# jlko/STOVE

Hardware: AMD Instinct MI355X
Metric: frames/s (fwd+bwd) for 3-obj billiards 32x32 T=100, 1/2/4/8 GPU; ELBO delta vs ref (higher is better)
Workload: dtype f32 (encoder GEMMs: fp32 products as 3 sixteen-bit MFMAs on hi/lo-split operands -- half pieces forward, bf16 pieces backward -- fp32 accumulate)

## Files before the change

### stove_amd/csrc/capi.hip

```cpp
#include "../../include/stove_hip.h"
#include <algorithm>

#include "common.h"
#include <string.h>
#include <stdlib.h>
#include <math.h>
#include <atomic>
#include <type_traits>
#include "validate.h"
static_assert(stove_validate::kStoveInvalidValue == (int)hipErrorInvalidValue, "validate.h returns hipErrorInvalidValue");
#define STOVE_VALIDATE(expr)                      \
  do {                                            \
    const int v__ = stove_validate::expr;         \
    if (v__) return v__;                          \
  } while (0)
#include "spn_obj.hip"
#include "spn_obj_generic.hip"
#include "spn_bg.hip"
#include "spn_bg_generic.hip"
#include "scene.hip"
#include "scene_fused.hip"
#include "scene_colour.hip"
#include "gnn.hip"
#include "match.hip"
// ... 1266 lines not shown
  *graph_out = (void*)g;
  return (int)e;
}

int stove_graph_instantiate(void* graph, void** exec_out) {
  if (exec_out == nullptr) return (int)hipErrorInvalidValue;
  *exec_out = nullptr;
  if (graph == nullptr) return 0;
  hipGraph_t g = (hipGraph_t)graph;
  size_t n = 0;
  hipError_t e = hipGraphGetNodes(g, nullptr, &n);
  if (e == hipSuccess && n > 0) {
    hipGraphExec_t x = nullptr;
    e = hipGraphInstantiate(&x, g, nullptr, nullptr, 0);
    if (e == hipSuccess) *exec_out = (void*)x;
  }
  const hipError_t d = hipGraphDestroy(g);
  return (int)(e != hipSuccess ? e : d);
}

int stove_graph_launch(void* exec, void* stream) { return (int)hipGraphLaunch((hipGraphExec_t)exec, (hipStream_t)stream); }

int stove_graph_destroy(void* exec) { return exec == nullptr ? 0 : (int)hipGraphExecDestroy((hipGraphExec_t)exec); }

int stove_bw_transform(const float* x, float* out, int n_frames, int channels, int pixels, void* stream) {
  if (n_frames == 0) return 0;
  if (pixels % 4 != 0 || channels < 1) return (int)hipErrorInvalidValue;
  const long long total = (long long)n_frames * (pixels / 4);
  if (total > 0x7fffffffLL) return (int)hipErrorInvalidValue;
  STOVE_LAUNCH(bw_transform_k, dim3((unsigned)((total + 255) / 256)), dim3(256), 0, (hipStream_t)stream, x, out, n_frames, channels, pixels / 4);
  STOVE_LAUNCH_CHECK();
  return 0;
}

int stove_bw_transform_u8(const unsigned char* x, float* out, int n_frames, int channels, int pixels, void* stream) {
  if (n_frames == 0) return 0;
  if (pixels % 4 != 0 || channels < 1) return (int)hipErrorInvalidValue;
  const long long total = (long long)n_frames * (pixels / 4);
  if (total > 0x7fffffffLL) return (int)hipErrorInvalidValue;
  STOVE_LAUNCH(bw_transform_u8_k, dim3((unsigned)((total + 255) / 256)), dim3(256), 0, (hipStream_t)stream, x, out, n_frames, channels, pixels / 4);
  STOVE_LAUNCH_CHECK();
  return 0;
}

size_t stove_colsum_ws_floats(int rows, int cols) {
  const int chunks = rows < 512 ? (rows < 1 ? 1 : rows) : 512;
  return (size_t)(chunks + 16) * cols;
}

static int colsum_level(const float* a, float* part, int rows, int cols, int max_chunks, hipStream_t st) {
  const int chunks = rows < max_chunks ? rows : max_chunks;
  const int per = (rows + chunks - 1) / chunks;
  const int used = (rows + per - 1) / per;
  if (cols <= 64) {
    int cpad = 1;
    while (cpad < cols) cpad <<= 1;
    STOVE_LAUNCH(colsum_narrow_part_k, dim3(used), dim3(256), 0, st, a, part, rows, cols, cpad, per);
  } else {
    STOVE_LAUNCH(colsum_part_k, dim3(used, (cols / 4 + 255) / 256), dim3(256), 0, st, a, part, rows, cols / 4, per);
  }
  return used;
}

int stove_colsum(const float* a, float* out, float* ws, int rows, int cols, void* stream) { return stove_colsum2(a, out, nullptr, 0, ws, rows, cols, stream); }

int stove_colsum2(const float* a, float* out, float* out2, int accumulate, float* ws, int rows, int cols, void* stream) {
  hipStream_t st = (hipStream_t)stream;
  if (cols <= 0 || (cols % 4 != 0 && cols > 64)) return (int)hipErrorInvalidValue;
  if (rows == 0) {
    if (!accumulate) {
      hipMemsetAsync(out, 0, sizeof(float) * cols, st);
      if (out2 != nullptr) hipMemsetAsync(out2, 0, sizeof(float) * cols, st);
    }
    return 0;
  }
  int used = colsum_level(a, ws, rows, cols, 512, st);
  STOVE_LAUNCH_CHECK();
  const float* src = ws;
  if (used > 16) {
    float* ws2 = ws + (size_t)(rows < 512 ? rows : 512) * cols;
    used = colsum_level(ws, ws2, used, cols, 16, st);
    STOVE_LAUNCH_CHECK();
    src = ws2;
  }
  STOVE_LAUNCH(reduce_chunks_k, dim3((cols + 31) / 32), dim3(256), 0, st, src, out, cols, used, accumulate, out2);
  STOVE_LAUNCH_CHECK();
  return 0;
}

static int small_tn_chunks(int rows) { return rows < 64 ? 1 : (rows / 64 < 512 ? rows / 64 : 512); }
size_t stove_small_tn_ws_floats(int rows, int M, int N) { return (size_t)small_tn_chunks(rows) * M * N; }

int stove_small_tn(const float* a, const float* b, float* out, float* ws, int rows, int M, int N, void* stream) {
  hipStream_t st = (hipStream_t)stream;
  if (M < 1 || N < 1 || M * N > 256) return (int)hipErrorInvalidValue;
  if (rows == 0) {
    hipMemsetAsync(out, 0, sizeof(float) * M * N, st);
    return 0;
  }
  const int chunks = small_tn_chunks(rows), per = (rows + chunks - 1) / chunks;
  STOVE_LAUNCH(small_tn_part_k, dim3(chunks), dim3(256), 0, st, a, b, ws, rows, M, N, per);
  STOVE_LAUNCH_CHECK();
  STOVE_LAUNCH(reduce_chunks_k, dim3((M * N + 31) / 32), dim3(256), 0, st, (const float*)ws, out, M * N, chunks, 0);
  STOVE_LAUNCH_CHECK();
  return 0;
}

size_t stove_flat_adam_ws_bytes(int nseg) { return (size_t)nseg * sizeof(int) + ADAM_SCAN_BLOCKS * sizeof(float); }

int stove_flat_adam(float* params, const float* grads, float* exp_avg, float* exp_avg_sq, float* max_exp_avg_sq, size_t numel,
                    const int* seg_of4, const unsigned char* seg_trainable, float* seg_steps, int nseg, void* ws, float* grad_norm_out,
                    const float* hyper_dev, float lr, float beta1, float beta2, float eps, float max_norm, int clip, void* stream) {
  if (numel == 0 || nseg == 0) return 0;
  if (numel % 4 != 0 || ws == nullptr || seg_of4 == nullptr || seg_trainable == nullptr || seg_steps == nullptr)
    return (int)hipErrorInvalidValue;
  AdamHyper k;
  k.lr = lr; k.b1 = beta1; k.b2 = beta2; k.eps = eps; k.max_norm = max_norm;
  const int n4 = (int)(numel / 4);
  hipStream_t st = (hipStream_t)stream;
  float* part = reinterpret_cast<float*>(ws);
  int* flags = reinterpret_cast<int*>(part + ADAM_SCAN_BLOCKS);
  STOVE_LAUNCH(grad_scan_k, dim3(ADAM_SCAN_BLOCKS), dim3(256), 0, st, grads, seg_of4, flags, part, n4);
  STOVE_LAUNCH(flat_adam_k, dim3((n4 + 255) / 256), dim3(256), 0, st, params, grads, exp_avg, exp_avg_sq, max_exp_avg_sq, seg_of4,
               seg_trainable, (const float*)seg_steps, (const int*)flags, (const float*)part, grad_norm_out, hyper_dev, k, clip & 1, n4);
  STOVE_LAUNCH(adam_tick_k, dim3((nseg + 255) / 256), dim3(256), 0, st, seg_trainable, seg_steps, flags, nseg, (clip >> 1) & 1);
  STOVE_LAUNCH_CHECK();
  return 0;
}

static ZpConst zp_const(const float* span_low) {
  ZpConst k;
  for (int d = 0; d < 8; ++d) {
    k.span[d] = span_low[d];
    k.low[d] = span_low[8 + d];
  }
  return k;
}

int stove_supair_state_fwd(const float* codes, const float* span_low, float* zc, float* pos, long long* idx, float* zfix,
                           unsigned char* hits, float* zl, float* sl, float* init6, int n, int T, int o, int skip, int fix,
                           int mode, void* stream) {
  return stove_supair_state_fwd2(codes, span_low, zc, pos, idx, zfix, hits, zl, sl, init6, 6, nullptr, 0, n, T, o, skip, fix, mode, stream);
}

int stove_supair_state_fwd2(const float* codes, const float* span_low, float* zc, float* pos, long long* idx, float* zfix,
                            unsigned char* hits, float* zl, float* sl, float* init, int init_ld, const float* lat_noise, int lat_dim,
                            int n, int T, int o, int skip, int fix, int mode, void* stream) {
  if (init_ld < 6 + (lat_noise != nullptr ? lat_dim : 0) || lat_dim < 0) return (int)hipErrorInvalidValue;
  float* init6 = init;
  hipStream_t st = (hipStream_t)stream;
  if (n == 0) return 0;
  if (T < 2 || skip < 1 || skip >= T || o < 1 || o > kMatchN) return (int)hipErrorInvalidValue;
  const int M = n * T * o;
  if (codes != nullptr) {
    STOVE_LAUNCH(zp_constrain_k, dim3((M * 8 + 255) / 256), dim3(256), 0, st, codes, zp_const(span_low), zc, pos, M);
    STOVE_LAUNCH_CHECK();
    int rc = stove_match_objects(pos, idx, nullptr, n, T, o, 2, mode, stream);
    if (rc) return rc;
  }
  STOVE_LAUNCH(supair_state_fwd_k, dim3((M + 255) / 256), dim3(256), 0, st, (const float*)zc, (const long long*)idx, zfix, hits, zl, sl,
               init6, n, T, o, skip, fix, init_ld, lat_noise, lat_dim);
  STOVE_LAUNCH_CHECK();
  return 0;
}

int stove_supair_state_bwd(const float* zc, const long long* idx, const unsigned char* hits, const float* zfix, const float* g_zfix,
                           const float* g_zl, const float* g_sl, const float* g_init6, const float* span_low, float* gfix_ws,
                           float* g_codes, int n, int T, int o, int skip, void* stream) {
  return stove_supair_state_bwd2(zc, idx, hits, zfix, g_zfix, g_zl, g_sl, g_init6, 6, span_low, gfix_ws, g_codes, n, T, o, skip, stream);
}

int stove_supair_state_bwd2(const float* zc, const long long* idx, const unsigned char* hits, const float* zfix, const float* g_zfix,
                            const float* g_zl, const float* g_sl, const float* g_init6, int init_ld, const float* span_low, float* gfix_ws,
                            float* g_codes, int n, int T, int o, int skip, void* stream) {
  hipStream_t st = (hipStream_t)stream;
  if (n == 0) return 0;
  const int M = n * T * o;
  (void)gfix_ws;
  STOVE_LAUNCH(supair_state_bwd_k, dim3((M + 255) / 256), dim3(256), 0, st, zc, idx, hits, zfix, g_zfix, g_zl, g_sl, g_init6, zp_const(span_low),
               g_codes, n, T, o, skip, init_ld);
  STOVE_LAUNCH_CHECK();
  return 0;
}

int stove_noise_normal(float* out, size_t n, unsigned long long* state, void* stream) {
  if (n == 0) return 0;
  if (((uintptr_t)out & 15) != 0 || state == nullptr) return (int)hipErrorInvalidValue;
  const size_t threads = (n + 3) / 4;
  if ((threads + 255) / 256 > 0x7fffffffULL) return (int)hipErrorInvalidValue;
  STOVE_LAUNCH(noise_normal_k, dim3((unsigned)((threads + 255) / 256)), dim3(256), 0, (hipStream_t)stream, out, n, (const unsigned long long*)state);
  STOVE_LAUNCH(noise_tick_k, dim3(1), dim3(1), 0, (hipStream_t)stream, state);
  STOVE_LAUNCH_CHECK();
  return 0;
}

int stove_zall_fwd(const float* zfix, const float* zs, float* zall, int n, int T, int o, int skip, void* stream) {
  if (n == 0) return 0;
  const int M = n * (T - 1) * o;
  STOVE_LAUNCH(zall_fwd_k, dim3((M + 255) / 256), dim3(256), 0, (hipStream_t)stream, zfix, zs, zall, n, T, o, skip);
  STOVE_LAUNCH_CHECK();
  return 0;
}

int stove_zall_bwd(const float* zfix, const float* zs, const float* g_zall, const float* dz_in, float* g_zfix, float* g_zs, int n, int T, int o,
                   int skip, void* stream) {
  if (n == 0) return 0;
  const int M = n * T * o + n * (T - skip) * o;
  STOVE_LAUNCH(zall_bwd_k, dim3((M + 255) / 256), dim3(256), 0, (hipStream_t)stream, zfix, zs, g_zall, dz_in, g_zfix, g_zs, n, T, o, skip);
  STOVE_LAUNCH_CHECK();
  return 0;
}

static TransStd trans_std(const float* s16) {
  TransStd t;
  for (int d = 0; d < 16; ++d) t.s[d] = s16[d];
  return t;
}

int stove_elbo_fwd(const float* zs, const float* mean, const float* std_, const float* zdyn, const float* lik, const float* trans_std16,
                   float* part_ws, float* out3, int n, int T, int o, int skip, void* stream) {
  hipStream_t st = (hipStream_t)stream;
  if (n == 0 || skip < 1 || skip >= T) return (int)hipErrorInvalidValue;
  STOVE_LAUNCH(elbo_part_k, dim3(n), dim3(256), 0, st, zs, mean, std_, zdyn, lik, trans_std(trans_std16), part_ws, T, o, skip);
  STOVE_LAUNCH_CHECK();
  STOVE_LAUNCH(elbo_final_k, dim3(1), dim3(256), 0, st, (const float*)part_ws, out3, n, T, skip);
  STOVE_LAUNCH_CHECK();
  return 0;
}

int stove_elbo_bwd(const float* zs, const float* mean, const float* std_, const float* zdyn, const float* trans_std16, const float* g_out,
                   float* g_zs, float* g_mean, float* g_std, float* g_zdyn, float* g_lik, int n, int T, int o, int skip, void* stream) {
  if (n == 0) return 0;
  const size_t M = (size_t)n * (T - skip) * o * 18 + (size_t)n * (T - 1);
  STOVE_LAUNCH(elbo_bwd_k, dim3((unsigned)((M + 255) / 256)), dim3(256), 0, (hipStream_t)stream, zs, mean, std_, zdyn, trans_std(trans_std16), g_out,
               g_zs, g_mean, g_std, g_zdyn, g_lik, n, T, o, skip);
  STOVE_LAUNCH_CHECK();
  return 0;
}

static int enc_head_groups(int rows) {
  const int tiles = (rows + 15) / 16;
  int g = (tiles + 3) / 4;
  return g < 1 ? 1 : (g > 102 ? 102 : g);
}

int stove_enc_head_fwd(const float* h, const float* W1, const float* b1, const float* W2, const float* b2, float* h1, float* codes, int rows,
                       int H, int HID, int OUT, int frames, int fc1_split, void* stream) {
  if (H != kEhH || HID < 1 || HID > kEhHid || OUT != kEhOut || frames < 0 || (frames > 0 && rows % frames != 0)) return (int)hipErrorInvalidValue;
  if (rows == 0) return 0;
  static_assert(2 * kEhHid * kEhLdB == sizeof(float) * kEhHid * kEhLd, "the two bf16 images of W1 take the fp32 image's place");
  const size_t lds = sizeof(float) * kEhHid * kEhLd;
  const int tiles = (rows + 15) / 16;
  const int grid = (tiles + 3) / 4 < 512 ? (tiles + 3) / 4 : 512;
  int rc;
  if (fc1_split) {
    rc = (int)hipFuncSetAttribute((const void*)enc_head_fwd_k<true>, hipFuncAttributeMaxDynamicSharedMemorySize, (int)lds);
    if (rc) return rc;
    STOVE_LAUNCH((enc_head_fwd_k<true>), dim3(grid), dim3(256), lds, (hipStream_t)stream, h, W1, b1, W2, b2, h1, codes, rows, HID, frames);
  } else {
    rc = (int)hipFuncSetAttribute((const void*)enc_head_fwd_k<false>, hipFuncAttributeMaxDynamicSharedMemorySize, (int)lds);
    if (rc) return rc;
    STOVE_LAUNCH((enc_head_fwd_k<false>), dim3(grid), dim3(256), lds, (hipStream_t)stream, h, W1, b1, W2, b2, h1, codes, rows, HID, frames);
  }
  STOVE_LAUNCH_CHECK();
  return 0;
}

size_t stove_enc_head_bwd_ws_floats(int rows, int HID) { return (size_t)enc_head_groups(rows) * eh_part_floats(HID); }

int stove_enc_head_bwd(const float* dcodes, const float* h1, const float* h, const float* W1, const float* W2, float* gh, float* gW1,
                       float* gb1, float* gW2, float* gb2, int accumulate, float* ws, int rows, int H, int HID, int OUT, int frames, void* stream) {
  if (H != kEhH || HID < 1 || HID > kEhHid || OUT != kEhOut || frames < 0 || (frames > 0 && rows % frames != 0)) return (int)hipErrorInvalidValue;
  hipStream_t st = (hipStream_t)stream;
  const int P = eh_part_floats(HID);
  if (rows == 0) {
    if (!accumulate) {
      hipMemsetAsync(gW1, 0, sizeof(float) * HID * kEhH, st);
      hipMemsetAsync(gW2, 0, sizeof(float) * kEhOut * HID, st);
      hipMemsetAsync(gb1, 0, sizeof(float) * HID, st);
      hipMemsetAsync(gb2, 0, sizeof(float) * kEhOut, st);
    }
    return 0;
  }
  const int groups = enc_head_groups(rows);
  const size_t lds = sizeof(float) * kEhBwdLds;
  int rc;
  if (HID <= 50) {
    rc = (int)hipFuncSetAttribute((const void*)enc_head_bwd_k<14>, hipFuncAttributeMaxDynamicSharedMemorySize, (int)lds);
    if (rc) return rc;
    STOVE_LAUNCH(enc_head_bwd_k<14>, dim3(groups * 5), dim3(256), lds, st, dcodes, h1, h, W1, W2, gh, ws, rows, HID, groups, frames);
  } else {
    rc = (int)hipFuncSetAttribute((const void*)enc_head_bwd_k<16>, hipFuncAttributeMaxDynamicSharedMemorySize, (int)lds);
    if (rc) return rc;
    STOVE_LAUNCH(enc_head_bwd_k<16>, dim3(groups * 5), dim3(256), lds, st, dcodes, h1, h, W1, W2, gh, ws, rows, HID, groups, frames);
  }
  STOVE_LAUNCH_CHECK();
  (void)P;
  STOVE_LAUNCH(enc_head_reduce_k, dim3((eh_part_floats(HID) + 31) / 32), dim3(256), 0, st, (const float*)ws, gW1, gW2, gb1, gb2, HID, groups, accumulate);
  STOVE_LAUNCH_CHECK();
  return 0;
}

int stove_lstm_cell_fwd(const float* gx, const float* gh, const float* c_prev, float* c, float* h, int n, int H, int fast, void* stream) {
  if (n == 0) return 0;
  if (H % 4) return (int)hipErrorInvalidValue;
  const size_t total = (size_t)n * (H / 4);
// ... 116 lines not shown
```

### stove_amd/csrc/match.hip

```cpp
#include "common.h"

namespace stove {

constexpr int kMatchN = 8, kMatchF = 8;

template <int TN, int TF>
__global__ __launch_bounds__(64) void match_objects_k(const float* __restrict__ feat, long long* __restrict__ idx_out,
                                                      float* __restrict__ perm_out, int B, int T, int Nrt, int Frt, int mode) {
  const int N = TN > 0 ? TN : Nrt;
  const int F = TF > 0 ? TF : Frt;
  extern __shared__ float mlds[];
  const int b = blockIdx.x;
  const int n_feat = T * N * F;
  int* ibuf = reinterpret_cast<int*>(mlds + n_feat);
  for (int i = threadIdx.x; i < n_feat; i += 64) mlds[i] = feat[(size_t)b * n_feat + i];
  __syncthreads();
  if (threadIdx.x == 0) {
  constexpr int MN = TN > 0 ? TN : kMatchN, MF = TF > 0 ? TF : kMatchF;
  float prev[MN][MF], cur[MN][MF], err[MN][MN];
  const float* fb = mlds;
  _Pragma("unroll") for (int a = 0; a < N; ++a) {
    _Pragma("unroll") for (int f = 0; f < F; ++f) prev[a][f] = (fb[a * F + f] + 1.0f) * 0.5f;
    ibuf[a] = a;
  }
// ... 156 lines not shown
    e = fmaf(d, d, e);
  }
  return e;
}
__device__ __forceinline__ bool greedy_rounds(float (&e)[kMatchN][kMatchN], int N, int* assign) {
  bool tie = false;
  for (int round = 0; round < N; ++round) {
    float bv = __builtin_inff();
    int ba = 0, bj = 0, cnt = 0;
#pragma unroll
    for (int a = 0; a < kMatchN; ++a)
#pragma unroll
      for (int j = 0; j < kMatchN; ++j) {
        if (a < N && j < N) {
          const float v = e[a][j];
          cnt = v < bv ? 1 : (v == bv ? cnt + 1 : cnt);
          if (v < bv) {
            bv = v;
            ba = a;
            bj = j;
          }
        }
      }
    tie = tie || (cnt > 1 && bv < 3.0e38f);
    assign[ba] = bj;
#pragma unroll
    for (int a = 0; a < kMatchN; ++a)
#pragma unroll
      for (int j = 0; j < kMatchN; ++j)
        if (a == ba || j == bj) e[a][j] = 3.0e38f;
  }
  return tie;
}
__device__ __forceinline__ unsigned char* greedy_scratch(long long* idx_out, int b, int T, int N) {
  return reinterpret_cast<unsigned char*>(idx_out + (size_t)(b + 1) * T * N) - (size_t)T * N - T;
}
__global__ __launch_bounds__(256) void match_greedy_frames_k(const float* __restrict__ feat, long long* __restrict__ idx_out, int B, int T, int N, int F) {
  const int i = blockIdx.x * blockDim.x + threadIdx.x;
  if (i >= B * T) return;
  const int b = i / T, t = i % T;
  unsigned char* sc = greedy_scratch(idx_out, b, T, N);
  if (t == 0) {
    for (int a = 0; a < N; ++a) sc[a] = (unsigned char)a;
    sc[(size_t)T * N] = 0;
    return;
  }
  const float* prev = feat + ((size_t)b * T + t - 1) * N * F;
  const float* cur = prev + (size_t)N * F;
  float e[kMatchN][kMatchN];
#pragma unroll
  for (int a = 0; a < kMatchN; ++a)
#pragma unroll
    for (int j = 0; j < kMatchN; ++j) e[a][j] = (a < N && j < N) ? match_err(prev + a * F, cur + j * F, F) : 3.0e38f;
  int assign[kMatchN];
#pragma unroll
  for (int a = 0; a < kMatchN; ++a) assign[a] = 0;
  const bool tie = greedy_rounds(e, N, assign);
#pragma unroll
  for (int a = 0; a < kMatchN; ++a)
    if (a < N) sc[(size_t)t * N + a] = (unsigned char)assign[a];
  sc[(size_t)T * N + t] = tie ? 1 : 0;
}
__global__ __launch_bounds__(64) void match_greedy_compose_k(const float* __restrict__ feat, long long* __restrict__ idx_out, int B, int T, int N, int F) {
  extern __shared__ unsigned char glds[];
  const int b = blockIdx.x, lane = threadIdx.x;
  const unsigned char* sc = greedy_scratch(idx_out, b, T, N);
  const int nsc = T * N + T;
  for (int i = lane; i < nsc; i += 64) glds[i] = sc[i];
  int* ibuf = reinterpret_cast<int*>(glds + ((nsc + 3) & ~3));
  __shared__ int slot[kMatchN];
  __syncthreads();
  int r = lane < N ? lane : 0;
  if (lane < N) ibuf[lane] = r;
  for (int t = 1; t < T; ++t) {
    if (glds[T * N + t] == 0) {
      r = glds[t * N + r];
    } else {
      if (lane < N) slot[lane] = r;
      __syncthreads();
      if (lane == 0) {
        const float* prev = feat + ((size_t)b * T + t - 1) * N * F;
        const float* cur = prev + (size_t)N * F;
        float e[kMatchN][kMatchN];
#pragma unroll
        for (int a = 0; a < kMatchN; ++a)
#pragma unroll
          for (int j = 0; j < kMatchN; ++j) e[a][j] = (a < N && j < N) ? match_err(prev + slot[a < N ? a : 0] * F, cur + j * F, F) : 3.0e38f;
        int assign[kMatchN];
#pragma unroll
        for (int a = 0; a < kMatchN; ++a) assign[a] = 0;
        greedy_rounds(e, N, assign);
#pragma unroll
        for (int a = 0; a < kMatchN; ++a)
          if (a < N) slot[a] = assign[a];
      }
      __syncthreads();
      if (lane < N) r = slot[lane];
      __syncthreads();
    }
    if (lane < N) ibuf[t * N + lane] = r;
  }
  __syncthreads();
  for (int i = lane; i < T * N; i += 64) idx_out[(size_t)b * T * N + i] = ibuf[i];
}

struct Perm3 {
  int p0, p1, p2;
};
__device__ __forceinline__ Perm3 perm3_of(int k) {
  Perm3 r;
  r.p0 = k >> 1;
  const int lo = r.p0 == 0 ? 1 : 0, hi = r.p0 == 2 ? 1 : 2;
  r.p1 = (k & 1) ? hi : lo;
  r.p2 = (k & 1) ? lo : hi;
  return r;
}
__device__ __forceinline__ int perm3_id(const Perm3& p) { return 2 * p.p0 + (p.p1 > p.p2 ? 1 : 0); }
__device__ __forceinline__ float sel3(int i, float a, float b, float c) { return i == 0 ? a : (i == 1 ? b : c); }
__device__ __forceinline__ Perm3 match3_step(const float (&D)[3][3], const Perm3& p) {
  float e[3][3];
#pragma unroll
  for (int j = 0; j < 3; ++j) {
    e[0][j] = sel3(p.p0, D[0][j], D[1][j], D[2][j]);
    e[1][j] = sel3(p.p1, D[0][j], D[1][j], D[2][j]);
    e[2][j] = sel3(p.p2, D[0][j], D[1][j], D[2][j]);
  }
  int idx[3];
#pragma unroll
  for (int a = 0; a < 3; ++a) {
    int best = 0;
    if (e[a][1] < e[a][best]) best = 1;
    if (e[a][2] < sel3(best, e[a][0], e[a][1], e[a][2])) best = 2;
    idx[a] = best;
  }
  if (idx[0] == idx[1] || idx[0] == idx[2] || idx[1] == idx[2]) {
#pragma unroll
    for (int a = 0; a < 3; ++a) {
      int best = 0;
      if (e[a][1] < e[a][0]) best = 1;
      if (e[a][2] < sel3(best, e[a][0], e[a][1], e[a][2])) best = 2;
      idx[a] = best;
#pragma unroll
      for (int r = 0; r < 3; ++r) {
        e[r][0] = best == 0 ? 1e12f : e[r][0];
        e[r][1] = best == 1 ? 1e12f : e[r][1];
        e[r][2] = best == 2 ? 1e12f : e[r][2];
      }
    }
  }
  return Perm3{idx[0], idx[1], idx[2]};
}

template <int F>
__global__ __launch_bounds__(64) void match3_table_k(const float* __restrict__ feat, long long* __restrict__ idx_out, int B, int T) {
  extern __shared__ float mlds[];
  const int b = blockIdx.x, lane = threadIdx.x;
  const int n_feat = T * 3 * F;
  int* ibuf = reinterpret_cast<int*>(mlds + n_feat);
  for (int i = lane; i < n_feat; i += 64) mlds[i] = feat[(size_t)b * n_feat + i];
  __syncthreads();
  const int chunk = (T - 1 + 63) / 64;
  const int t0 = 1 + lane * chunk, t1 = t0 + chunk < T ? t0 + chunk : T;
  auto table = [&](int t, float (&D)[3][3]) {
    float pv[3][F], cv[3][F];
#pragma unroll
    for (int i = 0; i < 3; ++i)
#pragma unroll
      for (int f = 0; f < F; ++f) {
        pv[i][f] = (mlds[((t - 1) * 3 + i) * F + f] + 1.0f) * 0.5f;
        cv[i][f] = (mlds[(t * 3 + i) * F + f] + 1.0f) * 0.5f;
      }
#pragma unroll
    for (int i = 0; i < 3; ++i)
#pragma unroll
      for (int j = 0; j < 3; ++j) {
        float sacc = 0.0f;
#pragma unroll
        for (int f = 0; f < F; ++f) {
          const float d = pv[i][f] - cv[j][f];
          sacc += d * d;
        }
        D[i][j] = sacc;
      }
  };
  int cur[6] = {0, 1, 2, 3, 4, 5};
  for (int t = t0; t < t1; ++t) {
    float D[3][3];
    table(t, D);
#pragma unroll
    for (int k = 0; k < 6; ++k) cur[k] = perm3_id(match3_step(D, perm3_of(cur[k])));
  }
  unsigned m = 0;
#pragma unroll
  for (int k = 0; k < 6; ++k) m |= (unsigned)cur[k] << (3 * k);
#pragma unroll
  for (int d = 1; d < 64; d <<= 1) {
    const unsigned o = (unsigned)__builtin_amdgcn_ds_bpermute(((lane - d) & 63) * 4, (int)m);
    if (lane >= d) {
      unsigned n = 0;
#pragma unroll
      for (int k = 0; k < 6; ++k) n |= ((m >> (3 * ((o >> (3 * k)) & 7u))) & 7u) << (3 * k);
      m = n;
    }
  }
  const unsigned before = (unsigned)__builtin_amdgcn_ds_bpermute(((lane - 1) & 63) * 4, (int)m);
  Perm3 p = perm3_of(lane == 0 ? 0 : (int)(before & 7u));
  if (lane == 0) {
    ibuf[0] = 0;
    ibuf[1] = 1;
    ibuf[2] = 2;
  }
  for (int t = t0; t < t1; ++t) {
    float D[3][3];
    table(t, D);
    p = match3_step(D, p);
    ibuf[t * 3 + 0] = p.p0;
    ibuf[t * 3 + 1] = p.p1;
    ibuf[t * 3 + 2] = p.p2;
  }
  __syncthreads();
  for (int i = lane; i < T * 3; i += 64) idx_out[(size_t)b * T * 3 + i] = ibuf[i];
}

}
```

### stove_amd/csrc/state.hip

```cpp
#include "common.h"

namespace stove {

struct ZpConst {
  float span[8], low[8];
};

__global__ void zp_constrain_k(const float* __restrict__ codes, ZpConst kc, float* __restrict__ zc, float* __restrict__ pos, int M) {
  const int i = blockIdx.x * blockDim.x + threadIdx.x;
  if (i >= M * 8) return;
  const int d = i & 7;
  const float v = fmaf(kc.span[d], sigmoidf_(codes[i]), kc.low[d]);
  zc[i] = v;
  if (d == 2 || d == 3) pos[(i >> 3) * 2 + d - 2] = v;
}

__device__ __forceinline__ void load8(const float* __restrict__ p, float* v) {
  const float4 a = *reinterpret_cast<const float4*>(p), b = *reinterpret_cast<const float4*>(p + 4);
  v[0] = a.x; v[1] = a.y; v[2] = a.z; v[3] = a.w; v[4] = b.x; v[5] = b.y; v[6] = b.z; v[7] = b.w;
}

__device__ __forceinline__ int fixed_state(const float* __restrict__ zc, const long long* __restrict__ idx, int b, int t, int k, int T,
                                           int o, int fix, float* out) {
  const size_t row = (size_t)b * T + t;
  float cur[8];
  load8(zc + (row * o + idx[row * o + k]) * 8, cur);
  int hit = 0;
  if (fix && t >= 1 && t <= T - 2) {
    float pv[8], nx[8];
    load8(zc + ((row - 1) * o + idx[(row - 1) * o + k]) * 8, pv);
    load8(zc + ((row + 1) * o + idx[(row + 1) * o + k]) * 8, nx);
#pragma unroll
    for (int a = 0; a < 2; ++a)
      if (fabsf(cur[a] - pv[a]) > 0.095f && fabsf(nx[a] - cur[a]) > 0.095f) hit |= 1 << a;
#pragma unroll
    for (int d = 0; d < 8; ++d)
      if (hit & (1 << (d & 1))) cur[d] = 0.5f * (pv[d] + nx[d]);
  }
#pragma unroll
  for (int d = 0; d < 8; ++d) out[d] = cur[d];
  return hit;
}

__global__ void supair_state_fwd_k(const float* __restrict__ zc, const long long* __restrict__ idx, float* __restrict__ zfix,
                                   unsigned char* __restrict__ hits, float* __restrict__ zl, float* __restrict__ sl,
                                   float* __restrict__ init6, int n, int T, int o, int skip, int fix, int init_ld,
                                   const float* __restrict__ lat_noise, int lat_dim) {
  const int i = blockIdx.x * blockDim.x + threadIdx.x;
  if (i >= n * T * o) return;
  const int k = i % o, t = (i / o) % T, b = i / (o * T);
  float cur[8], pv[8];
  const int hit = fixed_state(zc, idx, b, t, k, T, o, fix, cur);
  hits[i] = (unsigned char)hit;
#pragma unroll
  for (int d = 0; d < 8; ++d) zfix[(size_t)i * 8 + d] = cur[d];
  if (t < skip - 1 || t < 1) return;
  fixed_state(zc, idx, b, t - 1, k, T, o, fix, pv);
  float z6[6], s6[6];
#pragma unroll
  for (int d = 0; d < 4; ++d) {
    z6[d] = cur[d];
    s6[d] = cur[4 + d];
  }
#pragma unroll
  for (int a = 0; a < 2; ++a) {
    z6[4 + a] = cur[2 + a] - pv[2 + a];
    s6[4 + a] = sqrtf(cur[6 + a] * cur[6 + a] + pv[6 + a] * pv[6 + a]);
  }
  if (t == skip - 1) {
#pragma unroll
    for (int d = 0; d < 6; ++d) init6[((size_t)b * o + k) * init_ld + d] = z6[d];
    if (lat_noise != nullptr)
      for (int d = 0; d < lat_dim; ++d) init6[((size_t)b * o + k) * init_ld + 6 + d] = 0.01f * lat_noise[((size_t)b * o + k) * lat_dim + d];
  } else {
    const size_t r = (((size_t)b * (T - skip) + (t - skip)) * o + k) * 6;
#pragma unroll
    for (int d = 0; d < 6; ++d) {
      zl[r + d] = z6[d];
      sl[r + d] = s6[d];
    }
  }
}

__device__ __forceinline__ void g6_at(const float* __restrict__ g_zl, const float* __restrict__ g_sl, const float* __restrict__ g_init6,
                                      int b, int t, int k, int T, int o, int skip, float* gz, float* gs, int init_ld) {
#pragma unroll
  for (int d = 0; d < 6; ++d) gz[d] = gs[d] = 0.0f;
  if (t < 1 || t > T - 1) return;
  if (t == skip - 1) {
    if (g_init6 != nullptr)
#pragma unroll
      for (int d = 0; d < 6; ++d) gz[d] = g_init6[((size_t)b * o + k) * init_ld + d];
  } else if (t >= skip) {
    const size_t r = (((size_t)b * (T - skip) + (t - skip)) * o + k) * 6;
#pragma unroll
    for (int d = 0; d < 6; ++d) {
      if (g_zl != nullptr) gz[d] = g_zl[r + d];
      if (g_sl != nullptr) gs[d] = g_sl[r + d];
    }
  }
}

__device__ __forceinline__ void supair_gfix(const float* __restrict__ zfix, const float* __restrict__ g_zfix, const float* __restrict__ g_zl,
                                            const float* __restrict__ g_sl, const float* __restrict__ g_init6, size_t i, int T, int o, int skip,
                                            int init_ld, float (&g)[8]) {
  const int k = (int)(i % o), t = (int)((i / o) % T), b = (int)(i / ((size_t)o * T));
#pragma unroll
  for (int d = 0; d < 8; ++d) g[d] = g_zfix != nullptr ? g_zfix[i * 8 + d] : 0.0f;
  float gz[6], gs[6], gzn[6], gsn[6];
  g6_at(g_zl, g_sl, g_init6, b, t, k, T, o, skip, gz, gs, init_ld);
  g6_at(g_zl, g_sl, g_init6, b, t + 1, k, T, o, skip, gzn, gsn, init_ld);
#pragma unroll
  for (int d = 0; d < 4; ++d) {
    g[d] += gz[d];
    g[4 + d] += gs[d];
  }
  float cur[8];
  load8(zfix + i * 8, cur);
#pragma unroll
  for (int a = 0; a < 2; ++a) {
    g[2 + a] += gz[4 + a] - gzn[4 + a];
    if (gs[4 + a] != 0.0f) {
      const float p = zfix[(i - o) * 8 + 6 + a];
      g[6 + a] += gs[4 + a] * cur[6 + a] / sqrtf(cur[6 + a] * cur[6 + a] + p * p);
    }
    if (gsn[4 + a] != 0.0f) {
      const float q = zfix[(i + o) * 8 + 6 + a];
      g[6 + a] += gsn[4 + a] * cur[6 + a] / sqrtf(q * q + cur[6 + a] * cur[6 + a]);
    }
  }
}

__global__ void supair_state_bwd_k(const float* __restrict__ zc, const long long* __restrict__ idx, const unsigned char* __restrict__ hits,
                                   const float* __restrict__ zfix, const float* __restrict__ g_zfix, const float* __restrict__ g_zl,
                                   const float* __restrict__ g_sl, const float* __restrict__ g_init6, ZpConst kc, float* __restrict__ g_codes,
                                   int n, int T, int o, int skip, int init_ld) {
  const int i = blockIdx.x * blockDim.x + threadIdx.x;
  if (i >= n * T * o) return;
  const int j = i % o, t = (i / o) % T, b = i / (o * T);
  const size_t row = (size_t)b * T + t;
  float acc[8] = {0, 0, 0, 0, 0, 0, 0, 0};
  for (int k = 0; k < o; ++k) {
    if ((int)idx[row * o + k] != j) continue;
    const size_t e = row * o + k;
    const int h0 = hits[e];
    const int hp = (t >= 1) ? hits[e - o] : 0, hn = (t <= T - 2) ? hits[e + o] : 0;
    float g0[8], gp[8], gn[8];
    supair_gfix(zfix, g_zfix, g_zl, g_sl, g_init6, e, T, o, skip, init_ld, g0);
    if (hp) supair_gfix(zfix, g_zfix, g_zl, g_sl, g_init6, e - o, T, o, skip, init_ld, gp);
    if (hn) supair_gfix(zfix, g_zfix, g_zl, g_sl, g_init6, e + o, T, o, skip, init_ld, gn);
#pragma unroll
    for (int d = 0; d < 8; ++d) {
      const int bit = 1 << (d & 1);
      float v = (h0 & bit) ? 0.0f : g0[d];
      if (hp & bit) v += 0.5f * gp[d];
      if (hn & bit) v += 0.5f * gn[d];
      acc[d] += v;
    }
  }
#pragma unroll
  for (int d = 0; d < 8; ++d) {
    const float s = (zc[(size_t)i * 8 + d] - kc.low[d]) / kc.span[d];
    g_codes[(size_t)i * 8 + d] = acc[d] * kc.span[d] * s * (1.0f - s);
  }
}

__global__ void zall_fwd_k(const float* __restrict__ zfix, const float* __restrict__ zs, float* __restrict__ zall, int n, int T, int o, int skip) {
  const int i = blockIdx.x * blockDim.x + threadIdx.x;
  if (i >= n * (T - 1) * o) return;
  const int k = i % o, j = (i / o) % (T - 1), b = i / (o * (T - 1));
  const float* src = (j < skip - 1) ? zfix + (((size_t)b * T + 1 + j) * o + k) * 8 : zs + (((size_t)b * (T - skip) + (j - (skip - 1))) * o + k) * 18;
  const float sx = src[0];
  zall[(size_t)i * 4] = sx;
  zall[(size_t)i * 4 + 1] = sx * src[1];
  zall[(size_t)i * 4 + 2] = src[2];
  zall[(size_t)i * 4 + 3] = src[3];
}
__global__ void zall_bwd_k(const float* __restrict__ zfix, const float* __restrict__ zs, const float* __restrict__ g_zall,
                           const float* __restrict__ dz_in, float* __restrict__ g_zfix, float* __restrict__ g_zs, int n, int T, int o, int skip) {
  const int i = blockIdx.x * blockDim.x + threadIdx.x;
  const int nfix = n * T * o, nzs = n * (T - skip) * o;
  if (i < nfix) {
    const int k = i % o, t = (i / o) % T, b = i / (o * T);
    float g[8] = {0, 0, 0, 0, 0, 0, 0, 0};
    if (t >= 1 && t < skip) {
      const size_t a = (((size_t)b * (T - 1) + (t - 1)) * o + k) * 4;
      const float* src = zfix + (size_t)i * 8;
      g[0] = g_zall[a] + g_zall[a + 1] * src[1];
      g[1] = g_zall[a + 1] * src[0];
      g[2] = g_zall[a + 2];
      g[3] = g_zall[a + 3];
    }
#pragma unroll
    for (int d = 0; d < 8; ++d) g_zfix[(size_t)i * 8 + d] = g[d];
  } else if (i < nfix + nzs) {
    const int q = i - nfix;
    const int k = q % o, ts = (q / o) % (T - skip), b = q / (o * (T - skip));
    const size_t a = (((size_t)b * (T - 1) + (skip - 1 + ts)) * o + k) * 4;
    const float* src = zs + (size_t)q * 18;
    float* g = g_zs + (size_t)q * 18;
    float v[4];
    v[0] = g_zall[a] + g_zall[a + 1] * src[1];
    v[1] = g_zall[a + 1] * src[0];
    v[2] = g_zall[a + 2];
    v[3] = g_zall[a + 3];
    if (dz_in == nullptr) {
#pragma unroll
      for (int d = 0; d < 18; ++d) g[d] = d < 4 ? v[d] : 0.0f;
    } else {
      const float* gi = dz_in + (size_t)q * 18;
#pragma unroll
      for (int d = 0; d < 18; ++d) g[d] = d < 4 ? v[d] + gi[d] : gi[d];
    }
  }
}

__device__ __forceinline__ void philox_round(uint32_t& c0, uint32_t& c1, uint32_t& c2, uint32_t& c3, uint32_t k0, uint32_t k1) {
  const uint64_t p0 = (uint64_t)0xD2511F53u * c0, p1 = (uint64_t)0xCD9E8D57u * c2;
  const uint32_t n0 = (uint32_t)(p1 >> 32) ^ c1 ^ k0, n2 = (uint32_t)(p0 >> 32) ^ c3 ^ k1;
  c1 = (uint32_t)p1;
  c3 = (uint32_t)p0;
  c0 = n0;
  c2 = n2;
}
__device__ __forceinline__ float u01(uint32_t r) { return ((float)(r >> 8) + 0.5f) * (1.0f / 16777216.0f); }
__global__ __launch_bounds__(256) void noise_normal_k(float* __restrict__ out, size_t n, const unsigned long long* __restrict__ state) {
  const size_t i = (size_t)blockIdx.x * blockDim.x + threadIdx.x;
  if (4 * i >= n) return;
  const unsigned long long seed = state[0], call = state[1];
  uint32_t c0 = (uint32_t)call, c1 = (uint32_t)(call >> 32), c2 = (uint32_t)i, c3 = (uint32_t)(i >> 32);
  uint32_t k0 = (uint32_t)seed, k1 = (uint32_t)(seed >> 32);
#pragma unroll
  for (int r = 0; r < 10; ++r) {
// ... 108 lines not shown
```

Measured before the change: 9.099 million.

## Fuse zp constrain, 3-object matching and state fwd into one per-sequence kernel

For the 3-object, mode-0 case, a single kernel per batch element now computes the sigmoid constraint on the codes, keeps zc and pos in LDS, runs the 3-object table match walk on one wavefront, and builds the fixed states from LDS. Before, this took three separate launches with global round-trips for zc, pos and idx. The match walk is factored into a shared device function, and the state element code is templated on the index type so it can read the int LDS buffer. The cost is one block per sequence with only 64 of 256 threads active during matching, which may lower parallelism for small n.

```diff
diff --git a/stove_amd/csrc/capi.hip b/stove_amd/csrc/capi.hip
--- a/stove_amd/csrc/capi.hip
+++ b/stove_amd/csrc/capi.hip
@@ -1442,6 +1442,12 @@
   if (n == 0) return 0;
   if (T < 2 || skip < 1 || skip >= T || o < 1 || o > kMatchN) return (int)hipErrorInvalidValue;
   const int M = n * T * o;
+  if (codes != nullptr && mode == 0 && o == 3 && state3_lds_bytes(T) <= 64 * 1024) {
+    STOVE_LAUNCH(supair_state3_fwd_k, dim3(n), dim3(kState3Threads), state3_lds_bytes(T), st, codes, zp_const(span_low), zc, pos, idx, zfix, hits,
+                 zl, sl, init6, T, skip, fix, init_ld, lat_noise, lat_dim);
+    STOVE_LAUNCH_CHECK();
+    return 0;
+  }
   if (codes != nullptr) {
     STOVE_LAUNCH(zp_constrain_k, dim3((M * 8 + 255) / 256), dim3(256), 0, st, codes, zp_const(span_low), zc, pos, M);
     STOVE_LAUNCH_CHECK();
diff --git a/stove_amd/csrc/match.hip b/stove_amd/csrc/match.hip
--- a/stove_amd/csrc/match.hip
+++ b/stove_amd/csrc/match.hip
@@ -332,13 +332,7 @@
 }
 
 template <int F>
-__global__ __launch_bounds__(64) void match3_table_k(const float* __restrict__ feat, long long* __restrict__ idx_out, int B, int T) {
-  extern __shared__ float mlds[];
-  const int b = blockIdx.x, lane = threadIdx.x;
-  const int n_feat = T * 3 * F;
-  int* ibuf = reinterpret_cast<int*>(mlds + n_feat);
-  for (int i = lane; i < n_feat; i += 64) mlds[i] = feat[(size_t)b * n_feat + i];
-  __syncthreads();
+__device__ __forceinline__ void match3_table_walk(const float* mlds, int* ibuf, int T, int lane) {
   const int chunk = (T - 1 + 63) / 64;
   const int t0 = 1 + lane * chunk, t1 = t0 + chunk < T ? t0 + chunk : T;
   auto table = [&](int t, float (&D)[3][3]) {
@@ -398,6 +392,17 @@
     ibuf[t * 3 + 1] = p.p1;
     ibuf[t * 3 + 2] = p.p2;
   }
+}
+
+template <int F>
+__global__ __launch_bounds__(64) void match3_table_k(const float* __restrict__ feat, long long* __restrict__ idx_out, int B, int T) {
+  extern __shared__ float mlds[];
+  const int b = blockIdx.x, lane = threadIdx.x;
+  const int n_feat = T * 3 * F;
+  int* ibuf = reinterpret_cast<int*>(mlds + n_feat);
+  for (int i = lane; i < n_feat; i += 64) mlds[i] = feat[(size_t)b * n_feat + i];
+  __syncthreads();
+  match3_table_walk<F>(mlds, ibuf, T, lane);
   __syncthreads();
   for (int i = lane; i < T * 3; i += 64) idx_out[(size_t)b * T * 3 + i] = ibuf[i];
 }
diff --git a/stove_amd/csrc/state.hip b/stove_amd/csrc/state.hip
--- a/stove_amd/csrc/state.hip
+++ b/stove_amd/csrc/state.hip
@@ -20,7 +20,8 @@
   v[0] = a.x; v[1] = a.y; v[2] = a.z; v[3] = a.w; v[4] = b.x; v[5] = b.y; v[6] = b.z; v[7] = b.w;
 }
 
-__device__ __forceinline__ int fixed_state(const float* __restrict__ zc, const long long* __restrict__ idx, int b, int t, int k, int T,
+template <typename IdxT>
+__device__ __forceinline__ int fixed_state(const float* __restrict__ zc, const IdxT* __restrict__ idx, int b, int t, int k, int T,
                                            int o, int fix, float* out) {
   const size_t row = (size_t)b * T + t;
   float cur[8];
@@ -42,20 +43,19 @@
   return hit;
 }
 
-__global__ void supair_state_fwd_k(const float* __restrict__ zc, const long long* __restrict__ idx, float* __restrict__ zfix,
-                                   unsigned char* __restrict__ hits, float* __restrict__ zl, float* __restrict__ sl,
-                                   float* __restrict__ init6, int n, int T, int o, int skip, int fix, int init_ld,
-                                   const float* __restrict__ lat_noise, int lat_dim) {
-  const int i = blockIdx.x * blockDim.x + threadIdx.x;
-  if (i >= n * T * o) return;
-  const int k = i % o, t = (i / o) % T, b = i / (o * T);
+template <typename IdxT>
+__device__ __forceinline__ void supair_state_elem(const float* __restrict__ zc, const IdxT* __restrict__ idx, int bz, int b, int t, int k,
+                                                  float* __restrict__ zfix, unsigned char* __restrict__ hits, float* __restrict__ zl,
+                                                  float* __restrict__ sl, float* __restrict__ init6, int T, int o, int skip, int fix,
+                                                  int init_ld, const float* __restrict__ lat_noise, int lat_dim) {
+  const size_t i = ((size_t)b * T + t) * o + k;
   float cur[8], pv[8];
-  const int hit = fixed_state(zc, idx, b, t, k, T, o, fix, cur);
+  const int hit = fixed_state(zc, idx, bz, t, k, T, o, fix, cur);
   hits[i] = (unsigned char)hit;
 #pragma unroll
-  for (int d = 0; d < 8; ++d) zfix[(size_t)i * 8 + d] = cur[d];
+  for (int d = 0; d < 8; ++d) zfix[i * 8 + d] = cur[d];
   if (t < skip - 1 || t < 1) return;
-  fixed_state(zc, idx, b, t - 1, k, T, o, fix, pv);
+  fixed_state(zc, idx, bz, t - 1, k, T, o, fix, pv);
   float z6[6], s6[6];
 #pragma unroll
   for (int d = 0; d < 4; ++d) {
@@ -79,6 +79,50 @@
       zl[r + d] = z6[d];
       sl[r + d] = s6[d];
     }
+  }
+}
+
+__global__ void supair_state_fwd_k(const float* __restrict__ zc, const long long* __restrict__ idx, float* __restrict__ zfix,
+                                   unsigned char* __restrict__ hits, float* __restrict__ zl, float* __restrict__ sl,
+                                   float* __restrict__ init6, int n, int T, int o, int skip, int fix, int init_ld,
+                                   const float* __restrict__ lat_noise, int lat_dim) {
+  const int i = blockIdx.x * blockDim.x + threadIdx.x;
+  if (i >= n * T * o) return;
+  const int k = i % o, t = (i / o) % T, b = i / (o * T);
+  supair_state_elem(zc, idx, b, b, t, k, zfix, hits, zl, sl, init6, T, o, skip, fix, init_ld, lat_noise, lat_dim);
+}
+
+constexpr int kState3Threads = 256;
+__host__ __device__ inline size_t state3_lds_bytes(int T) { return (size_t)T * 3 * (8 + 2 + 1) * sizeof(float); }
+__global__ __launch_bounds__(kState3Threads) void supair_state3_fwd_k(const float* __restrict__ codes, ZpConst kc, float* __restrict__ zc,
+                                                                      float* __restrict__ pos, long long* __restrict__ idx_out,
+                                                                      float* __restrict__ zfix, unsigned char* __restrict__ hits,
+                                                                      float* __restrict__ zl, float* __restrict__ sl,
+                                                                      float* __restrict__ init6, int T, int skip, int fix, int init_ld,
+                                                                      const float* __restrict__ lat_noise, int lat_dim) {
+  extern __shared__ __attribute__((aligned(16))) float s3_lds[];
+  float* zc_s = s3_lds;
+  float* pos_s = zc_s + T * 3 * 8;
+  int* ibuf = reinterpret_cast<int*>(pos_s + T * 3 * 2);
+  const int b = blockIdx.x, tid = threadIdx.x;
+  const int M = T * 3;
+  const size_t row0 = (size_t)b * M;
+  for (int i = tid; i < M * 8; i += kState3Threads) {
+    const int d = i & 7;
+    const float v = fmaf(kc.span[d], sigmoidf_(codes[row0 * 8 + i]), kc.low[d]);
+    zc[row0 * 8 + i] = v;
+    zc_s[i] = v;
+    if (d == 2 || d == 3) {
+      pos[(row0 + (i >> 3)) * 2 + d - 2] = v;
+      pos_s[(i >> 3) * 2 + d - 2] = v;
+    }
+  }
+  __syncthreads();
+  if (tid < 64) match3_table_walk<2>(pos_s, ibuf, T, tid);
+  __syncthreads();
+  for (int i = tid; i < M; i += kState3Threads) {
+    idx_out[row0 + i] = ibuf[i];
+    supair_state_elem(zc_s, ibuf, 0, b, i / 3, i % 3, zfix, hits, zl, sl, init6, T, 3, skip, fix, init_ld, lat_noise, lat_dim);
   }
 }
 
```

After: 9.131 million (median of 5 runs). Within noise of the previous version (+0.4%).
